# inai17ibar/video-diffusion-pipeline-parallel

Measured on AMD Instinct MI355X. Metric: steady-state videos/sec (whole node), SVD 14f x 25step, higher is better.
Workload: dtype f16

## Files before the change

### include/svdpipe.h

```cpp
#ifndef SVDPIPE_H
#define SVDPIPE_H

#include <stddef.h>
#include <stdint.h>

#ifdef __cplusplus
extern "C" {
#endif

#define SP_OK 0
#define SP_EINVAL (-1)
#define SP_ELAUNCH (-2)

const char *sp_last_error(void);
int sp_version(void);
#define SP_ZERO_PAGE_BYTES 4096

enum { SP_A_LINEAR = 0, SP_A_CONV3X3 = 1, SP_A_TEMPORAL3 = 2 };

typedef struct sp_gemm_desc {
  const void *a;
  int64_t lda;
  int mode;
  int cin;
// ... 33 lines not shown

const char *sp_gemm_last_kernel(void);

int sp_conv_up2x_f16(const void *a, int64_t lda, int cin, int n_img, int hin, int win, const void *w, int n,
                     const float *bias, void *d, int64_t ldd, float *gn_part, const void *zero_page, void *stream);

int sp_gemm_set_route(int route, int bm, int bn);

int sp_gemv_f16(const void *x, int64_t ldx, const void *w, const float *b, float *y, void *y_f16,
                int64_t ldy, int rows, int n, int k, int silu_in, int silu_out, void *stream);
int sp_gemv_batched_f16(const void *x, int64_t ldx, int64_t x_stride, const void *w, int64_t w_stride,
                        const float *b, int64_t b_stride, float *y, void *y_f16, int64_t ldy, int64_t y_stride,
                        int batch, int rows, int n, int k, int silu_in, int silu_out, void *stream);

int sp_sinusoid_f16(const float *values, void *out, int count, int dim, void *stream);

size_t sp_groupnorm_ws_bytes(int instances, int64_t rows, int c, int groups);
int sp_groupnorm_f16(const void *x, const float *gamma, const float *beta, void *y, int instances,
                     int64_t rows, int c, int groups, float eps, int fuse_silu, void *ws,
                     size_t ws_bytes, void *stream);
int sp_groupnorm_ld_f16(const void *x, int64_t ldx, const float *gamma, const float *beta, void *y, int instances,
                        int64_t rows, int c, int groups, float eps, int fuse_silu, void *ws,
                        size_t ws_bytes, void *stream);

int sp_groupnorm_tile_sums_f16(const void *x, int64_t ldx, const float *part, const float *gamma, const float *beta, void *y,
                               int instances, int64_t rows, int c, int groups, float eps, int fuse_silu, float *stats,
                               void *stream);
int sp_groupnorm_tile_sums2_f16(const void *x, int64_t ldx, const float *part, int c_a, const float *part_b, const float *gamma,
                                const float *beta, void *y, int instances, int64_t rows, int c, int groups, float eps,
                                int fuse_silu, float *stats, void *stream);
int sp_groupnorm_fold_linear_tile_sums_f16(const float *part, const float *gamma, const float *beta, int instances, int64_t rows,
                                           int c, int groups, float eps, const void *w, const float *bias, int n, void *w_out,
                                           float *bias_out, float *stats, void *stream);
int sp_groupnorm_fold_linear_f16(const void *x, int64_t ldx, const float *gamma, const float *beta, int instances,
                                 int64_t rows, int c, int groups, float eps, const void *w, const float *bias, int n,
                                 void *w_out, float *bias_out, void *ws, size_t ws_bytes, void *stream);

int sp_layernorm_f16(const void *x, const void *addvec, int64_t addvec_rows, void *sum_out,
                     const float *gamma, const float *beta, void *y, int64_t rows, int c, float eps,
                     void *stream);
int sp_ln_stats_f16(const void *x, const void *addvec, int64_t addvec_rows, void *sum_out, float *stats,
                    int64_t rows, int c, float eps, void *stream);

int sp_attn_spatial_f16(const void *q, const void *k, const void *v, void *o, int64_t ldq,
                        int64_t ldk, int64_t ldv, int64_t ldo, int batch, int seq, int heads,
                        float scale, const void *zero_page, void *stream);
int sp_attn_temporal_f16(const void *q, const void *k, const void *v, void *o, int64_t ldq,
                         int64_t ldk, int64_t ldv, int64_t ldo, int batch, int frames, int64_t hw,
                         int heads, float scale, const void *zero_page, void *stream);
int64_t sp_attn_long_ws_bytes(int batch, int seq, int heads);
int sp_attn_spatial_long_f16(const void *q, const void *k, const void *v, void *o, int64_t ldq, int64_t ldk,
                             int64_t ldv, int64_t ldo, int batch, int seq, int heads, float scale,
                             const void *zero_page, void *workspace, int64_t workspace_bytes, void *stream);
int64_t sp_attn_fp8_ws_bytes(int batch, int seq, int heads);
int sp_attn_spatial_fp8(const void *q, const void *k, const void *v, void *o, int64_t ldq, int64_t ldk,
                        int64_t ldv, int64_t ldo, int batch, int seq, int heads, float scale,
                        void *workspace, int64_t workspace_bytes, const void *zero_page, void *stream);

int sp_pack_input_f16(const void *latent, const void *image_latents, void *out, float in_scale,
                      int b, int frames, int h, int w, int cpad, void *stream);
int sp_euler_step_f16(const void *latent, const void *eps_cond, const void *eps_uncond,
                      int64_t ld_eps, const float *guidance , void *out, float sigma,
                      float sigma_next, int b, int frames, int h, int w, void *stream);
int sp_euler_step_rows_f16(const void *latent, const void *eps_cond, const void *eps_uncond,
                           int64_t ld_eps, const float *guidance, int64_t ld_guidance, void *out, float sigma,
                           float sigma_next, int b, int frames, int h, int w, void *stream);
int sp_dpmpp2m_step_rows_f16(const void *state, const void *eps_cond, const void *eps_uncond,
                             int64_t ld_eps, const float *guidance, int64_t ld_guidance, void *out_state,
                             float sigma, float a, float b, float c1, float c2,
                             int batch, int frames, int h, int w, void *stream);
int sp_concat_channels_f16(const void *a, int ca, const void *b, int cb, void *out, int64_t rows,
                           void *stream);
int sp_add_rowvec_f16(const void *x, const float *vec, void *y, int64_t rows, int c, void *stream);

int sp_softmax_rows_f16(void *x, int64_t ld, int64_t rows, int cols, void *stream);
int sp_gemm_f32out_f16(const void *a, int64_t lda, const void *w, void *d, int m, int n, int k, const void *zero_page,
                       void *stream);
int sp_softmax_rows_f32(const float *x, int64_t ld, void *out, int64_t ldo, int64_t rows, int cols, float scale, void *stream);
int sp_vae_pack_latent_f16(const void *latent, void *rows, float scale, int64_t flat0, int n, int F, int64_t sb,
                           int64_t sc, int64_t sf, int h, int w, int cpad, void *stream);
int sp_vae_frames_out_f16(const void *rows, int64_t ld, const float *weight, const float *bias, void *out,
                          int out_fp32, int batch, int frames, int h, int w, int64_t flat0, int F, int64_t sb,
                          int64_t sc, int64_t sf, void *stream);
int sp_vae_frames_out_u8(const void *rows, int64_t ld, const float *weight, const float *bias, void *out, int batch,
                         int frames, int h, int w, int64_t flat0, void *stream);

int sp_vae_image_pack_f16(const void *image, void *rows, int batch, int h, int w, int cpad, int flip, void *stream);
int sp_vae_latent_out_f16(const void *rows, int64_t ld, void *out, int batch, int channels, int frames, int h, int w,
                          int flip, void *stream);

int sp_patchify_f16(const void *pixels, void *rows, int batch, int h, int w, int patch, int kpad, void *stream);
int sp_attn_small_f16(const void *q, const void *k, const void *v, void *o, int64_t ldq, int64_t ldk, int64_t ldv,
                      int64_t ldo, int batch, int seq, int heads, int head_dim, float scale, void *stream);
int sp_gelu_f16(const void *x, void *y, int64_t n, int quick, void *stream);

enum { SP_FILTER_BICUBIC = 0 , SP_FILTER_LANCZOS3 = 1  };
size_t sp_image_resample_tmp_bytes(int src_h, int dst_w);
int sp_image_resample_u8(const void *src, int64_t src_pitch, int src_h, int src_w, void *dst, int64_t dst_pitch, int dst_h,
                         int dst_w, int filter, void *tmp, size_t tmp_bytes, void *stream);
int sp_image_to_tensor_f16(const void *src, int64_t src_pitch, int h, int w, void *out, float mean0, float mean1, float mean2,
                           float std0, float std1, float std2, void *stream);
int sp_frames_to_u8(const void *frames, int is_fp32, void *out, int batch, int frames_n, int h, int w, void *stream);

int sp_jpeg_quant_tables(int quality, uint8_t *luma64, uint8_t *chroma64);
int sp_jpeg_huffman_table(int which, uint8_t *bits16, uint8_t *vals162);
size_t sp_jpeg_coef_bytes(int n, int h, int w);
// ... 59 lines not shown
```

### video-diffusion-pipeline-parallel_amd/csrc/attention_long.hip

```cpp
#include "common.h"

namespace {

typedef unsigned u32x4 __attribute__((ext_vector_type(4)));
typedef unsigned u32x2 __attribute__((ext_vector_type(2)));

__device__ __forceinline__ float fast_exp2(float x) { return __builtin_amdgcn_exp2f(x); }

constexpr unsigned LONG_BAIL_MIN = 64, LONG_BAIL_MAX = 512;

template <int QB>
__global__ __launch_bounds__(256, 1) void attn_long_kernel(
    const f16 *__restrict__ q, const f16 *__restrict__ k, const f16 *__restrict__ v, f16 *__restrict__ o,
    int64_t ldq, int64_t ldk, int64_t ldv, int64_t ldo, int seq, int heads, float scale_log2e,
    unsigned *__restrict__ flags) {
  constexpr int KV = 64;
  constexpr int K_BYTES = KV * 128, STAGE = 2 * K_BYTES, RING = 3;
  constexpr int OWN = 2 * QB;
  constexpr int WARM = OWN + 1;
  __shared__ __attribute__((aligned(16))) char smem[RING * STAGE];

  const int tid = threadIdx.x, lane = tid & 63;
  const int wave = __builtin_amdgcn_readfirstlane(tid >> 6);
  const int bh = blockIdx.y;
  {
    unsigned *const flagged_waves = flags + (int64_t)gridDim.x * gridDim.y;
    if (tid == 0) *(volatile unsigned *)smem = __hip_atomic_load(flagged_waves, __ATOMIC_RELAXED, __HIP_MEMORY_SCOPE_AGENT);
    __syncthreads();
    const unsigned seen = *(volatile unsigned *)smem;
    __syncthreads();
    const unsigned total_waves = gridDim.x * gridDim.y * 4u;
    const unsigned frac = total_waves / 16u;
    const unsigned bail = frac < LONG_BAIL_MIN ? LONG_BAIL_MIN : (frac > LONG_BAIL_MAX ? LONG_BAIL_MAX : frac);
    if (seen >= bail) {
      if (tid == 0) flags[(int64_t)bh * gridDim.x + blockIdx.x] = 1u;
      return;
    }
  }
  const int b = bh / heads, hd = bh - b * heads;
  const int r = lane & 31, h = lane >> 5;
  const int64_t row0 = (int64_t)b * seq;
  const int q0 = blockIdx.x * (128 * QB) + wave * (32 * QB);

  f16x8 qf[QB][4];
#pragma unroll
  for (int qb = 0; qb < QB; ++qb) {
    const f16 *qp = q + (row0 + q0 + qb * 32 + r) * ldq + hd * 64 + 8 * h;
#pragma unroll
    for (int s = 0; s < 4; ++s) {
      const f16x8 raw = *(const f16x8 *)(qp + 16 * s);
#pragma unroll
      for (int e = 0; e < 8; ++e) qf[qb][s][e] = (f16)((float)raw[e] * scale_log2e);
    }
  }

  const int lrow = lane >> 3, lchunk = lane & 7;
  unsigned kofl[2], vofl[2];
#pragma unroll
  for (int i = 0; i < 2; ++i) {
    const int row = wave * 16 + i * 8 + lrow;
    kofl[i] = (unsigned)((row * ldk + ((lchunk ^ ((row >> 1) & 7)) << 3)) * 2);
    vofl[i] = (unsigned)((row * ldv + ((lchunk ^ (((row >> 1) & 1) << 2)) << 3)) * 2);
  }
  const int64_t kstep = (int64_t)KV * ldk * 2, vstep = (int64_t)KV * ldv * 2;

  int koff[2];
#pragma unroll
  for (int kt = 0; kt < 2; ++kt) koff[kt] = (kt * 32 + r) * 128;
  int kswz = (r >> 1) & 7, hq = h;
  const int g = lane >> 4, i16 = lane & 15, q_ = i16 >> 2, pp = i16 & 3;
  const int vrow_l = 4 * (g >> 1) + q_;
  const int vchunk_l = 2 * (g & 1) + (pp >> 1);
  const int vswz = (q_ >> 1) << 2;
// ... 23 lines not shown

  const int own0 = blockIdx.x * OWN;
  const char *kbase = (const char *)(k + row0 * ldk + hd * 64);
  const char *vbase = (const char *)(v + row0 * ldv + hd * 64);
  auto stage = [&](int i, int buf) {
    const int tl = i < OWN ? own0 + i : (i - OWN < own0 ? i - OWN : i);
    const char *kb = kbase + tl * kstep, *vb = vbase + tl * vstep;
    char *sk = smem + buf * STAGE;
    char *sv = sk + K_BYTES;
#pragma unroll
    for (int j = 0; j < 2; ++j) {
      glds16(kb + kofl[j], sk + (wave * 16 + j * 8) * 128);
      glds16(vb + vofl[j], sv + (wave * 16 + j * 8) * 128);
    }
  };
  stage(0, 0);
  stage(1, 1);
  asm volatile("s_waitcnt vmcnt(4)" ::: "memory");
  __builtin_amdgcn_s_barrier();

  auto qk = [&](int qb, const char *sk, f32x16 (&sacc)[2]) {
    f16x8 kf[2][4];
#pragma unroll
    for (int kt = 0; kt < 2; ++kt)
#pragma unroll
      for (int s = 0; s < 4; ++s) kf[kt][s] = *(const f16x8 *)(sk + koff[kt] + (((2 * s + hq) ^ kswz) << 4));
#pragma unroll
    for (int kt = 0; kt < 2; ++kt)
#pragma unroll
      for (int s = 0; s < 4; ++s)
        sacc[kt] = __builtin_amdgcn_mfma_f32_32x32x16_f16(kf[kt][s], qf[qb][s], s == 0 ? negm[qb] : sacc[kt], 0, 0, 0);
  };
  auto pv = [&](int qb, const u32x4 (&pw)[2][2], const u32x2 (&vr)[2][8]) {
#pragma unroll
    for (int dt = 0; dt < 2; ++dt)
#pragma unroll
      for (int kt = 0; kt < 2; ++kt)
#pragma unroll
        for (int s = 0; s < 2; ++s) {
          const u32x4 vw = {vr[dt][4 * kt + 2 * s][0], vr[dt][4 * kt + 2 * s][1], vr[dt][4 * kt + 2 * s + 1][0],
                            vr[dt][4 * kt + 2 * s + 1][1]};
          oacc[qb][dt] = __builtin_amdgcn_mfma_f32_32x32x16_f16(__builtin_bit_cast(f16x8, vw),
                                                               __builtin_bit_cast(f16x8, pw[kt][s]), oacc[qb][dt], 0, 0, 0);
          if (dt == 0)
            lacc[qb] = __builtin_amdgcn_mfma_f32_16x16x32_f16(lsel, __builtin_bit_cast(f16x8, pw[kt][s]), lacc[qb], 0, 0, 0);
        }
  };

  auto warm_tile = [&](int i, int buf) {
    if (i + 2 < ntiles) stage(i + 2, buf >= 1 ? buf - 1 : RING - 1);
    const char *sk = smem + buf * STAGE;
    const char *sv = sk + K_BYTES;

    f32x16 sacc[2][2];
    u32x4 pw[2][2][2];
    qk(0, sk, sacc[0]);
    u32x2 vr[2][8];
    {
      const unsigned va[2] = {(unsigned)(uintptr_t)(const __attribute__((address_space(3))) char *)(sv + vlane0),
                              (unsigned)(uintptr_t)(const __attribute__((address_space(3))) char *)(sv + vlane1)};
#pragma unroll
      for (int dt = 0; dt < 2; ++dt)
#pragma unroll
        for (int j = 0; j < 8; ++j)
          asm volatile("ds_read_b64_tr_b16 %0, %1 offset:%2" : "=v"(vr[dt][j]) : "v"(va[dt]), "n"(j * 8 * 128) : "memory");
      asm volatile("s_waitcnt lgkmcnt(0)"
                   : "+v"(vr[0][0]), "+v"(vr[0][1]), "+v"(vr[0][2]), "+v"(vr[0][3]), "+v"(vr[0][4]), "+v"(vr[0][5]),
                     "+v"(vr[0][6]), "+v"(vr[0][7]), "+v"(vr[1][0]), "+v"(vr[1][1]), "+v"(vr[1][2]), "+v"(vr[1][3]),
                     "+v"(vr[1][4]), "+v"(vr[1][5]), "+v"(vr[1][6]), "+v"(vr[1][7])::"memory");
    }

#pragma unroll
    for (int qb = 0; qb < QB; ++qb) {
      f32x16(&sc)[2] = sacc[qb & 1];
      if (qb > 0) pv(qb - 1, pw[(qb - 1) & 1], vr);
      {
        float mt = fmaxf(fmaxf(sc[0][0], sc[0][1]), sc[0][2]);
#pragma unroll
        for (int e = 3; e < 31; e += 2) mt = fmaxf(fmaxf(mt, sc[e >> 4][e & 15]), sc[(e + 1) >> 4][(e + 1) & 15]);
        mt = fmaxf(mt, sc[1][15]);
        float ma = mt, mb = mt;
        asm volatile("s_nop 1\n\tv_permlane32_swap_b32 %0, %1" : "+v"(ma), "+v"(mb));
        mt = fmaxf(ma, mb);
        const float delta = i == 0 ? mt : fmaxf(mt, 0.f);
        if (__builtin_amdgcn_ballot_w64(delta != 0.f) != 0) {
          const float alpha = i == 0 ? 1.f : fast_exp2(-delta);
          lacc[qb][0] *= alpha;
#pragma unroll
          for (int e = 0; e < 16; ++e) { oacc[qb][0][e] *= alpha; oacc[qb][1][e] *= alpha; }
#pragma unroll
          for (int kt = 0; kt < 2; ++kt)
#pragma unroll
            for (int e = 0; e < 16; ++e) sc[kt][e] -= delta;
          m_run[qb] += delta;
#pragma unroll
          for (int e = 0; e < 16; ++e) negm[qb][e] = -m_run[qb];
        }
      }
      if (qb + 1 < QB) qk(qb + 1, sk, sacc[(qb + 1) & 1]);
      u32x4(&pc)[2][2] = pw[qb & 1];
#pragma unroll
      for (int kt = 0; kt < 2; ++kt)
#pragma unroll
        for (int e = 0; e < 16; e += 2) {
          const f32x2 p = {fast_exp2(sc[kt][e]), fast_exp2(sc[kt][e + 1])};
          pc[kt][e >> 3][(e & 7) >> 1] = __builtin_bit_cast(unsigned, __builtin_convertvector(p, f16x2));
// ... 98 lines not shown
#pragma unroll
    for (int s = 0; s < 4; ++s) { S(1, 1, s); Q(0, 1, 0, s); RV(s); SB(); }
    asm volatile("s_waitcnt lgkmcnt(0)"
                 : "+v"(vr[0][0]), "+v"(vr[0][1]), "+v"(vr[0][2]), "+v"(vr[0][3]), "+v"(vr[1][0]), "+v"(vr[1][1]), "+v"(vr[1][2]),
                   "+v"(vr[1][3])::"memory");
    SB();
    STAMP(3);
    P(0, 0, 0, 0); Q(0, 1, 1, 0); RV(4); SB();
    P(0, 0, 0, 1); Q(0, 1, 1, 1); RV(5); SB();
    P(0, 0, 0, 2); Q(0, 1, 1, 2); RV(6); SB();
    P(0, 0, 1, 0); Q(0, 1, 1, 3); RV(7); SB();
    P(0, 0, 1, 1); SB();
    P(0, 0, 1, 2); SB();
    asm volatile("s_waitcnt lgkmcnt(0)"
                 : "+v"(vr[0][4]), "+v"(vr[0][5]), "+v"(vr[0][6]), "+v"(vr[0][7]), "+v"(vr[1][4]), "+v"(vr[1][5]), "+v"(vr[1][6]),
                   "+v"(vr[1][7])::"memory");
    SB();
    STAMP(4);
    asm volatile("s_waitcnt vmcnt(2)" ::: "memory");
    __builtin_amdgcn_s_barrier();
    SB();
    STAMP(5);
#define ROW(pb, pkt, ps, qkt, qs, X0, X1, X2)                              \
    P(pb, pkt, ps, 0); Q(1, qkt, qs, 0); Q(1, qkt, qs, 1); X0; SB();       \
    P(pb, pkt, ps, 1); Q(1, qkt, qs, 2); X1; SB();                         \
    P(pb, pkt, ps, 2); Q(1, qkt, qs, 3); X2; SB();
    ROW(0, 1, 0, 0, 0, dma(1, false), , )
    ROW(0, 1, 1, 0, 1, dma(1, true), , )
    STAMP(6);
    ROW(1, 0, 0, 1, 0, RK(0), RK(1), RK(2))
    ROW(1, 0, 1, 1, 1, RK(3), RK(4), RK(5))
#undef ROW
    STAMP(7);
    P(1, 1, 0, 0); RK(6); SB();
    P(1, 1, 0, 1); RK(7); SB();
    P(1, 1, 0, 2); advance_global(); SB();
    P(1, 1, 1, 0); SB();
    P(1, 1, 1, 1); advance_slots(); SB();
    P(1, 1, 1, 2); SB();
    STAMP(8);
#undef SB
#undef STAMP
  };

  int buf = 0;
  for (int i = 0; i < WARM; ++i) {
    warm_tile(i, buf);
    buf = buf + 1 == RING ? 0 : buf + 1;
  }
#pragma unroll
  for (int qb = 0; qb < QB; ++qb)
#pragma unroll
    for (int s = 0; s < 4; ++s) asm volatile("" : "+v"(qf[qb][s]));
  asm volatile("" : "+v"(koff[0]), "+v"(koff[1]), "+v"(vlane0), "+v"(vlane1), "+v"(kofl[0]), "+v"(kofl[1]), "+v"(vofl[0]),
               "+v"(vofl[1]), "+v"(lsel), "+v"(kswz), "+v"(hq));
  read_k(buf);
#ifdef LONG_TRACE
  const unsigned long long tc0 = __builtin_amdgcn_s_memtime(), tw0 = wall_clock64();
#endif
  steady_setup(WARM, buf);
  for (int i = WARM; i < ntiles; ++i) steady2(i);
  asm volatile("s_waitcnt vmcnt(0)" ::: "memory");

#ifdef LONG_TRACE
  tr[14] = (unsigned)(__builtin_amdgcn_s_memtime() - tc0);
  tr[15] = (unsigned)(wall_clock64() - tw0);
  if (blockIdx.x == 3 && blockIdx.y == LONG_TRACE && tid < 16) flags[gridDim.x * gridDim.y + 1 + tid] = tr[tid];
#endif
  {
    bool bad = false;
#pragma unroll
    for (int qb = 0; qb < QB; ++qb) bad = bad || !(lacc[qb][0] < 3.0e38f);
    if (__builtin_amdgcn_ballot_w64(bad) != 0 && lane == 0) {
      flags[(int64_t)bh * gridDim.x + blockIdx.x] = 1u;
      __hip_atomic_fetch_add(flags + (int64_t)gridDim.x * gridDim.y, 1u, __ATOMIC_RELAXED, __HIP_MEMORY_SCOPE_AGENT);
    }
  }

#pragma unroll
  for (int qb = 0; qb < QB; ++qb) {
    const float inv = 1.0f / lacc[qb][0];
    f16 *op = o + (row0 + q0 + qb * 32 + r) * ldo + hd * 64 + 4 * h;
#pragma unroll
    for (int dt = 0; dt < 2; ++dt)
#pragma unroll
      for (int c = 0; c < 4; ++c) {
        f16x4 w;
#pragma unroll
        for (int e = 0; e < 4; ++e) w[e] = (f16)(oacc[qb][dt][4 * c + e] * inv);
        *(f16x4 *)(op + 32 * dt + 8 * c) = w;
      }
  }
}

}

constexpr int LONG_QB = 2;
constexpr int LONG_ROWS = 128 * LONG_QB;

int sp_attn_spatial_launch(const void *q, const void *k, const void *v, void *o, int64_t ldq, int64_t ldk, int64_t ldv,
                           int64_t ldo, int batch, int seq, int heads, float scale, const void *zero_page,
                           const unsigned *only_flagged, void *stream, const char *who);

extern "C" int64_t sp_attn_long_ws_bytes(int batch, int seq, int heads) {
  if (batch <= 0 || seq <= 0 || heads <= 0) return 0;
  return ((int64_t)batch * heads * ((seq + LONG_ROWS - 1) / LONG_ROWS) + 1) * (int64_t)sizeof(unsigned);
}

extern "C" int sp_attn_spatial_long_f16(const void *q, const void *k, const void *v, void *o, int64_t ldq, int64_t ldk,
                                        int64_t ldv, int64_t ldo, int batch, int seq, int heads, float scale,
                                        const void *zero_page, void *workspace, int64_t workspace_bytes, void *stream) {
  SP_REQUIRE(q && k && v && o && zero_page, "sp_attn_spatial_long_f16: null pointer");
  SP_REQUIRE(batch > 0 && seq > 0 && heads > 0, "sp_attn_spatial_long_f16: batch/seq/heads must be positive");
  if (!(seq >= 4096 && seq % LONG_ROWS == 0))
    return sp_attn_spatial_launch(q, k, v, o, ldq, ldk, ldv, ldo, batch, seq, heads, scale, zero_page, nullptr, stream,
                                  "sp_attn_spatial_long_f16");
  SP_REQUIRE(ldq % 8 == 0 && ldk % 8 == 0 && ldv % 8 == 0 && ldo % 4 == 0,
             "sp_attn_spatial_long_f16: strides must be multiples of 8");
  SP_REQUIRE((int64_t)batch * heads <= 65535, "sp_attn_spatial_long_f16: batch*heads too large");
  const int64_t need = sp_attn_long_ws_bytes(batch, seq, heads);
  SP_REQUIRE(workspace && ((uintptr_t)workspace & 3) == 0 && workspace_bytes >= need,
             "sp_attn_spatial_long_f16: workspace of %lld bytes, need %lld (4-byte aligned)", (long long)workspace_bytes,
             (long long)need);
  SP_REQUIRE(5 * 64 * ldk * 2 < (1ll << 31) && 5 * 64 * ldv * 2 < (1ll << 31), "sp_attn_spatial_long_f16: row stride too large");
  hipStream_t s = (hipStream_t)stream;
  unsigned *flags = (unsigned *)workspace;
  if (hipMemsetAsync(flags, 0, (size_t)need, s) != hipSuccess) {
    (void)hipGetLastError();
    sp_set_error("sp_attn_spatial_long_f16: hipMemsetAsync of the flag words failed");
    return SP_ELAUNCH;
  }
  SP_CLEAR_STALE_ERROR();
  hipLaunchKernelGGL(attn_long_kernel<LONG_QB>, dim3(seq / LONG_ROWS, batch * heads), dim3(256), 0, s, (const f16 *)q,
                     (const f16 *)k, (const f16 *)v, (f16 *)o, ldq, ldk, ldv, ldo, seq, heads, scale * 1.4426950408889634f,
                     flags);
  SP_CHECK_LAUNCH("sp_attn_spatial_long_f16");
  return sp_attn_spatial_launch(q, k, v, o, ldq, ldk, ldv, ldo, batch, seq, heads, scale, zero_page, flags, stream,
                                "sp_attn_spatial_long_f16(second pass)");
}
```

### video-diffusion-pipeline-parallel_amd/hip/__init__.py

```python

from __future__ import annotations

import ctypes
import os

_HERE = os.path.dirname(os.path.abspath(__file__))
LIB_PATH = os.path.join(_HERE, "libsvdpipe_hip.so")
_lib = None


class GemmDesc(ctypes.Structure):

    _fields_ = [
        ("a", ctypes.c_void_p), ("lda", ctypes.c_int64), ("mode", ctypes.c_int), ("cin", ctypes.c_int),
        ("n_img", ctypes.c_int), ("hin", ctypes.c_int), ("win", ctypes.c_int), ("hout", ctypes.c_int),
        ("wout", ctypes.c_int), ("stride", ctypes.c_int), ("upsample2x", ctypes.c_int),
        ("frames", ctypes.c_int), ("hw", ctypes.c_int64),
        ("w", ctypes.c_void_p), ("m", ctypes.c_int), ("n", ctypes.c_int),
        ("bias", ctypes.c_void_p), ("bias2", ctypes.c_void_p), ("bias2_rows", ctypes.c_int64),
        ("ldb2", ctypes.c_int64),
        ("res1", ctypes.c_void_p), ("ldr1", ctypes.c_int64), ("r1scale", ctypes.c_float),
        ("res2", ctypes.c_void_p), ("ldr2", ctypes.c_int64), ("r2scale", ctypes.c_float),
        ("oscale", ctypes.c_float), ("geglu", ctypes.c_int), ("n_store", ctypes.c_int),
        ("d", ctypes.c_void_p), ("ldd", ctypes.c_int64), ("zero_page", ctypes.c_void_p),
        ("ln_stats", ctypes.c_void_p), ("ln_colsum", ctypes.c_void_p),
        ("euler_latent", ctypes.c_void_p), ("euler_out", ctypes.c_void_p),
        ("euler_eps_uncond", ctypes.c_void_p), ("euler_ld_eps", ctypes.c_int64),
        ("euler_guidance", ctypes.c_void_p),
        ("euler_sigma", ctypes.c_float), ("euler_sigma_next", ctypes.c_float),
        ("euler_frames", ctypes.c_int), ("euler_hw", ctypes.c_int64),
        ("workspace", ctypes.c_void_p), ("workspace_bytes", ctypes.c_size_t),
        ("ln_out", ctypes.c_void_p), ("ln_out_eps", ctypes.c_float),
        ("w_group_rows", ctypes.c_int64), ("w_group_stride", ctypes.c_int64),
        ("gn_part", ctypes.c_void_p),
        ("a2", ctypes.c_void_p), ("lda2", ctypes.c_int64), ("cin2", ctypes.c_int),
        ("euler_guidance_ld", ctypes.c_int64),
    ]


_P, _I, _L, _F, _Z = ctypes.c_void_p, ctypes.c_int, ctypes.c_int64, ctypes.c_float, ctypes.c_size_t
SIGNATURES = {
    "sp_last_error": (ctypes.c_char_p, []),
    "sp_version": (_I, []),
    "sp_gemm_f16": (_I, [ctypes.POINTER(GemmDesc), _P]),
    "sp_gemm_desc_size": (_Z, []),
    "sp_gemm_workspace_bytes": (_Z, [ctypes.POINTER(GemmDesc)]),
    "sp_gemm_set_route": (_I, [_I, _I, _I]),
    "sp_gemm_last_kernel": (ctypes.c_char_p, []),
    "sp_conv_up2x_f16": (_I, [_P, _L, _I, _I, _I, _I, _P, _I, _P, _P, _L, _P, _P, _P]),
    "sp_gemv_f16": (_I, [_P, _L, _P, _P, _P, _P, _L, _I, _I, _I, _I, _I, _P]),
    "sp_gemv_batched_f16": (_I, [_P, _L, _L, _P, _L, _P, _L, _P, _P, _L, _L, _I, _I, _I, _I, _I, _I, _P]),
    "sp_sinusoid_f16": (_I, [_P, _P, _I, _I, _P]),
    "sp_groupnorm_ws_bytes": (_Z, [_I, _L, _I, _I]),
    "sp_groupnorm_f16": (_I, [_P, _P, _P, _P, _I, _L, _I, _I, _F, _I, _P, _Z, _P]),
    "sp_groupnorm_ld_f16": (_I, [_P, _L, _P, _P, _P, _I, _L, _I, _I, _F, _I, _P, _Z, _P]),
    "sp_groupnorm_tile_sums_f16": (_I, [_P, _L, _P, _P, _P, _P, _I, _L, _I, _I, _F, _I, _P, _P]),
    "sp_groupnorm_tile_sums2_f16": (_I, [_P, _L, _P, _I, _P, _P, _P, _P, _I, _L, _I, _I, _F, _I, _P, _P]),
    "sp_groupnorm_fold_linear_tile_sums_f16": (_I, [_P, _P, _P, _I, _L, _I, _I, _F, _P, _P, _I, _P, _P, _P, _P]),
    "sp_groupnorm_fold_linear_f16": (_I, [_P, _L, _P, _P, _I, _L, _I, _I, _F, _P, _P, _I, _P, _P, _P, _Z, _P]),
    "sp_layernorm_f16": (_I, [_P, _P, _L, _P, _P, _P, _P, _L, _I, _F, _P]),
    "sp_ln_stats_f16": (_I, [_P, _P, _L, _P, _P, _L, _I, _F, _P]),
    "sp_attn_spatial_f16": (_I, [_P, _P, _P, _P, _L, _L, _L, _L, _I, _I, _I, _F, _P, _P]),
    "sp_attn_long_ws_bytes": (_L, [_I, _I, _I]),
    "sp_attn_spatial_long_f16": (_I, [_P, _P, _P, _P, _L, _L, _L, _L, _I, _I, _I, _F, _P, _P, _L, _P]),
    "sp_attn_fp8_ws_bytes": (_L, [_I, _I, _I]),
    "sp_attn_spatial_fp8": (_I, [_P, _P, _P, _P, _L, _L, _L, _L, _I, _I, _I, _F, _P, _L, _P, _P]),
    "sp_attn_temporal_f16": (_I, [_P, _P, _P, _P, _L, _L, _L, _L, _I, _I, _L, _I, _F, _P, _P]),
    "sp_pack_input_f16": (_I, [_P, _P, _P, _F, _I, _I, _I, _I, _I, _P]),
    "sp_euler_step_f16": (_I, [_P, _P, _P, _L, _P, _P, _F, _F, _I, _I, _I, _I, _P]),
    "sp_euler_step_rows_f16": (_I, [_P, _P, _P, _L, _P, _L, _P, _F, _F, _I, _I, _I, _I, _P]),
    "sp_dpmpp2m_step_rows_f16": (_I, [_P, _P, _P, _L, _P, _L, _P, _F, _F, _F, _F, _F, _I, _I, _I, _I, _P]),
    "sp_concat_channels_f16": (_I, [_P, _I, _P, _I, _P, _L, _P]),
    "sp_add_rowvec_f16": (_I, [_P, _P, _P, _L, _I, _P]),
    "sp_softmax_rows_f16": (_I, [_P, _L, _L, _I, _P]),
    "sp_gemm_f32out_f16": (_I, [_P, _L, _P, _P, _I, _I, _I, _P, _P]),
    "sp_softmax_rows_f32": (_I, [_P, _L, _P, _L, _L, _I, _F, _P]),
    "sp_vae_pack_latent_f16": (_I, [_P, _P, _F, _L, _I, _I, _L, _L, _L, _I, _I, _I, _P]),
    "sp_vae_frames_out_f16": (_I, [_P, _L, _P, _P, _P, _I, _I, _I, _I, _I, _L, _I, _L, _L, _L, _P]),
    "sp_vae_frames_out_u8": (_I, [_P, _L, _P, _P, _P, _I, _I, _I, _I, _L, _P]),
    "sp_vae_image_pack_f16": (_I, [_P, _P, _I, _I, _I, _I, _I, _P]),
    "sp_vae_latent_out_f16": (_I, [_P, _L, _P, _I, _I, _I, _I, _I, _I, _P]),
    "sp_patchify_f16": (_I, [_P, _P, _I, _I, _I, _I, _I, _P]),
    "sp_attn_small_f16": (_I, [_P, _P, _P, _P, _L, _L, _L, _L, _I, _I, _I, _I, _F, _P]),
    "sp_gelu_f16": (_I, [_P, _P, _L, _I, _P]),
    "sp_image_resample_tmp_bytes": (_Z, [_I, _I]),
    "sp_image_resample_u8": (_I, [_P, _L, _I, _I, _P, _L, _I, _I, _I, _P, _Z, _P]),
    "sp_image_to_tensor_f16": (_I, [_P, _L, _I, _I, _P, _F, _F, _F, _F, _F, _F, _P]),
    "sp_frames_to_u8": (_I, [_P, _I, _P, _I, _I, _I, _I, _P]),
    "sp_jpeg_quant_tables": (_I, [_I, _P, _P]),
    "sp_jpeg_huffman_table": (_I, [_I, _P, _P]),
    "sp_jpeg_coef_bytes": (_Z, [_I, _I, _I]),
    "sp_jpeg_dct_quant_u8": (_I, [_P, _I, _I, _I, _I, _P, _P]),
    "sp_jpeg_stream_bytes": (_Z, [_I, _I, _I]),
    "sp_jpeg_entropy_ws_bytes": (_Z, [_I, _I, _I, _I]),
    "sp_jpeg_entropy": (_I, [_P, _I, _I, _I, _I, _P, _Z, _P, _P, _Z, _P]),
    "sp_jpeg_decode_plan_bytes": (_Z, []),
    "sp_jpeg_decode_plan": (_I, [_P, _P, _I, _P, _P, _I, _P]),
    "sp_jpeg_decode_ws_bytes": (_Z, [_P]),
    "sp_jpeg_decode_coef_bytes": (_Z, [_P]),
    "sp_jpeg_decode_split": (_I, [_P, _P, _P, _P, _Z, _P]),
    "sp_jpeg_decode_sync": (_I, [_P, _P, _P, _Z, _I, _I, _P]),
    "sp_jpeg_decode_coefficients": (_I, [_P, _P, _P, _Z, _I, _P, _P]),
    "sp_jpeg_decode_pixels": (_I, [_P, _P, _P, _Z, _P, _P, _P]),
    "sp_gif_ws_bytes": (_Z, [_I, _I, _I, _I]),
    "sp_gif_stream_bytes": (_Z, [_I, _I, _I]),
    "sp_gif_quantise_u8": (_I, [_P, _I, _I, _I, _P, _P, _P, _Z, _P]),
    "sp_gif_lzw": (_I, [_P, _I, _I, _I, _I, _P, _Z, _P, _P, _Z, _P]),
    "sp_png_ws_bytes": (_Z, [_I, _I, _I, _I]),
    "sp_png_stream_bytes": (_Z, [_I, _I, _I]),
    "sp_png_filter_u8": (_I, [_P, _I, _I, _I, _P, _P]),
    "sp_png_deflate": (_I, [_P, _I, _I, _I, _I, _P, _Z, _P, _P, _Z, _P]),
    "sp_png_file_bytes": (_Z, [_I, _I, _I]),
    "sp_apng_file_bytes": (_Z, [_I, _I, _I, _I]),
    "sp_png_wrap_ws_bytes": (_Z, [_I, _Z]),
    "sp_png_wrap": (_I, [_P, _Z, _P, _I, _I, _I, _I, _I, _I, _P, _Z, _P, _P, _Z, _P]),
    "sp_crc32_ws_bytes": (_Z, [_I, _Z]),
    "sp_crc32_rows": (_I, [_P, _Z, _P, _P, _I, _P, _P, _Z, _P]),
# ... 35 lines not shown
```

### video-diffusion-pipeline-parallel_amd/hip/ops.py

```python

from __future__ import annotations

import ctypes

import torch

from . import GemmDesc, last_error, load

A_LINEAR, A_CONV3X3, A_TEMPORAL3 = 0, 1, 2
ZERO_PAGE_BYTES = 4096
_zero_pages: dict = {}


class HipKernelError(RuntimeError):
    pass


PROFILE = None


class _Timed:
    def __init__(self, kind, flops, nbytes=0.0, tag=None):
        self.kind, self.flops, self.nbytes, self.tag = kind, flops, nbytes, tag

# ... 207 lines not shown


def groupnorm_fold_linear(x, gamma, beta, w, bias, w_out, bias_out, *, instances, rows, c, groups, eps, n, ws, ldx=None):
    with _Timed("groupnorm", 0.0, 2.0 * instances * rows * c + 2.0 * instances * n * c):
        ldx = int(c if ldx is None else ldx)
        if tuple(w_out.shape) != (instances, n, c) or not w_out.is_contiguous() or bias_out.dtype != torch.float32 \
                or tuple(bias_out.shape) != (instances, n) or not bias_out.is_contiguous():
            raise ValueError("groupnorm_fold_linear: w_out must be contiguous fp16 [instances][n][c], bias_out fp32 [instances][n]")
        _check(load().sp_groupnorm_fold_linear_f16(_rows(x, "x", ldx).data_ptr(), ldx, _ptr(gamma), _ptr(beta), instances,
                                                   rows, c, groups, eps, _f16(w, "w").data_ptr(), _ptr(bias), n,
                                                   _f16(w_out, "w_out").data_ptr(), bias_out.data_ptr(), ws.data_ptr(),
                                                   ws.numel() * ws.element_size(), _stream()), "sp_groupnorm_fold_linear_f16")
    return w_out, bias_out


def layernorm(x, gamma, beta, y, *, rows, c, eps=1e-5, addvec=None, addvec_rows=0, sum_out=None):
    with _Timed("layernorm", 0.0, (2 + (sum_out is not None)) * 2.0 * rows * c):
        _check(load().sp_layernorm_f16(_f16(x, "x").data_ptr(), _ptr(addvec), addvec_rows, _ptr(sum_out),
                                       gamma.data_ptr(), beta.data_ptr(), _f16(y, "y").data_ptr(), rows, c, eps,
                                       _stream()), "sp_layernorm_f16")
    return y


def ln_stats(x, stats, *, rows, c, eps=1e-5, addvec=None, addvec_rows=0, sum_out=None):
    with _Timed("ln_stats", 0.0, (1 + (sum_out is not None)) * 2.0 * rows * c + 8.0 * rows):
        _check(load().sp_ln_stats_f16(_f16(x, "x").data_ptr(), _ptr(addvec), addvec_rows, _ptr(sum_out),
                                      stats.data_ptr(), rows, c, eps, _stream()), "sp_ln_stats_f16")
    return stats


def attn_spatial(q, k, v, o, *, ldq, ldk, ldv, ldo, batch, seq, heads, scale=0.125):
    with _Timed("attn_spatial", 4.0 * batch * heads * seq * seq * 64):
        _check(load().sp_attn_spatial_f16(q.data_ptr(), k.data_ptr(), v.data_ptr(), o.data_ptr(), ldq, ldk, ldv, ldo,
                                          batch, seq, heads, scale, zero_page(o.device).data_ptr(), _stream()),
               "sp_attn_spatial_f16")
    return o


def attn_long_ws_bytes(batch, seq, heads) -> int:
    return int(load().sp_attn_long_ws_bytes(batch, seq, heads))


def attn_spatial_long(q, k, v, o, workspace, *, ldq, ldk, ldv, ldo, batch, seq, heads, scale=0.125):
    long_rows = seq >= 4096 and seq % 256 == 0
    with _Timed("attn_spatial_long" if long_rows else "attn_spatial", 4.0 * batch * heads * seq * seq * 64):
        _check(load().sp_attn_spatial_long_f16(q.data_ptr(), k.data_ptr(), v.data_ptr(), o.data_ptr(), ldq, ldk, ldv, ldo,
                                               batch, seq, heads, scale, zero_page(o.device).data_ptr(),
                                               workspace.data_ptr(), workspace.numel() * workspace.element_size(),
                                               _stream()),
               "sp_attn_spatial_long_f16")
    return o


def attn_fp8_ws_bytes(batch, seq, heads) -> int:
    return int(load().sp_attn_fp8_ws_bytes(batch, seq, heads))


def attn_spatial_fp8(q, k, v, o, workspace, *, ldq, ldk, ldv, ldo, batch, seq, heads, scale=0.125):
    with _Timed("attn_spatial", 4.0 * batch * heads * seq * seq * 64):
        _check(load().sp_attn_spatial_fp8(q.data_ptr(), k.data_ptr(), v.data_ptr(), o.data_ptr(), ldq, ldk, ldv, ldo,
                                          batch, seq, heads, scale, workspace.data_ptr(),
                                          workspace.numel() * workspace.element_size(),
                                          zero_page(o.device).data_ptr(), _stream()),
               "sp_attn_spatial_fp8")
    return o


def attn_temporal(q, k, v, o, *, ldq, ldk, ldv, ldo, batch, frames, hw, heads, scale=0.125):
    with _Timed("attn_temporal", 4.0 * batch * hw * heads * frames * frames * 64, 4 * 2.0 * batch * frames * hw * heads * 64):
        _check(load().sp_attn_temporal_f16(q.data_ptr(), k.data_ptr(), v.data_ptr(), o.data_ptr(), ldq, ldk, ldv, ldo,
                                           batch, frames, hw, heads, scale, zero_page(o.device).data_ptr(), _stream()),
               "sp_attn_temporal_f16")
    return o


def pack_input(latent, image_latents, out, *, in_scale, b, frames, h, w, cpad):
    _check(load().sp_pack_input_f16(_f16(latent, "latent").data_ptr(), _f16(image_latents, "image_latents").data_ptr(),
                                    out.data_ptr(), in_scale, b, frames, h, w, cpad, _stream()), "sp_pack_input_f16")
    return out


def softmax_rows(x, *, rows, cols, ld=None):
    ld = int(ld if ld is not None else cols)
    with _Timed("softmax_rows", 0.0, 2 * 2.0 * rows * cols):
        _check(load().sp_softmax_rows_f16(_rows(x, "x", ld).data_ptr(), ld, rows, cols, _stream()), "sp_softmax_rows_f16")
    return x


def gemm_f32out(a, w, out32, *, m, n, k, lda=None):
    lda = int(lda if lda is not None else a.stride(0))
    _f16(a, "a"); _f16(w, "w")
    if out32.dtype != torch.float32 or not out32.is_cuda or not out32.is_contiguous() or out32.numel() < m * n:
        raise TypeError("out32 must be a contiguous float32 HIP tensor of at least m*n elements")
    if w.dim() == 2 and w.shape[0] > 1 and w.stride(0) != k:
        raise ValueError(f"w: row stride {w.stride(0)} must equal k = {k}")
    with _Timed("gemm_f32out", 2.0 * m * n * k, 2.0 * (m * k + n * k) + 4.0 * m * n):
        _check(load().sp_gemm_f32out_f16(a.data_ptr(), lda, w.data_ptr(), out32.data_ptr(), m, n, k,
                                         zero_page(a.device).data_ptr(), _stream()), "sp_gemm_f32out_f16")
    return out32


def softmax_rows_f32(x32, out16, *, rows, cols, scale=1.0, ld=None, ldo=None):
    ld = int(ld if ld is not None else x32.stride(0))
    ldo = int(ldo if ldo is not None else out16.stride(0))
    if x32.dtype != torch.float32 or not x32.is_cuda or out16.dtype != torch.float16 or not out16.is_cuda:
        raise TypeError("x32 must be float32 and out16 float16, both on a HIP device")
# ... 504 lines not shown
```

Before: 0.8371.

## Run long spatial attention at two waves per SIMD with periodic early-bail checks

Templates the long attention kernel on occupancy and by default launches a variant with launch_bounds occupancy 2. That variant uses a simpler warm-up tile path, and every 32 tiles it checks for overflow and for the global bail counter so blocks can quit early to the fallback pass. The aim is to hide latency through more resident waves per SIMD, at the cost of tighter register budgets and a less hand-scheduled pipeline. It also adds a setter for the occupancy mode and a query that reports which kernel was last launched.

```diff
diff --git a/include/svdpipe.h b/include/svdpipe.h
--- a/include/svdpipe.h
+++ b/include/svdpipe.h
@@ -109,6 +109,8 @@
 int sp_attn_spatial_long_f16(const void *q, const void *k, const void *v, void *o, int64_t ldq, int64_t ldk,
                              int64_t ldv, int64_t ldo, int batch, int seq, int heads, float scale,
                              const void *zero_page, void *workspace, int64_t workspace_bytes, void *stream);
+int sp_attn_long_set_occupancy(int occ);
+const char *sp_attn_long_last_kernel(void);
 int64_t sp_attn_fp8_ws_bytes(int batch, int seq, int heads);
 int sp_attn_spatial_fp8(const void *q, const void *k, const void *v, void *o, int64_t ldq, int64_t ldk,
                         int64_t ldv, int64_t ldo, int batch, int seq, int heads, float scale,
diff --git a/video-diffusion-pipeline-parallel_amd/csrc/attention_long.hip b/video-diffusion-pipeline-parallel_amd/csrc/attention_long.hip
--- a/video-diffusion-pipeline-parallel_amd/csrc/attention_long.hip
+++ b/video-diffusion-pipeline-parallel_amd/csrc/attention_long.hip
@@ -8,9 +8,10 @@
 __device__ __forceinline__ float fast_exp2(float x) { return __builtin_amdgcn_exp2f(x); }
 
 constexpr unsigned LONG_BAIL_MIN = 64, LONG_BAIL_MAX = 512;
-
-template <int QB>
-__global__ __launch_bounds__(256, 1) void attn_long_kernel(
+constexpr int LONG_LOOK = 32;
+
+template <int QB, int OCC>
+__global__ __launch_bounds__(256, OCC) void attn_long_kernel(
     const f16 *__restrict__ q, const f16 *__restrict__ k, const f16 *__restrict__ v, f16 *__restrict__ o,
     int64_t ldq, int64_t ldk, int64_t ldv, int64_t ldo, int seq, int heads, float scale_log2e,
     unsigned *__restrict__ flags) {
@@ -18,7 +19,7 @@
   constexpr int K_BYTES = KV * 128, STAGE = 2 * K_BYTES, RING = 3;
   constexpr int OWN = 2 * QB;
   constexpr int WARM = OWN + 1;
-  __shared__ __attribute__((aligned(16))) char smem[RING * STAGE];
+  __shared__ __attribute__((aligned(16))) char smem[RING * STAGE + (OCC > 1 ? 32 : 0)];
 
   const int tid = threadIdx.x, lane = tid & 63;
   const int wave = __builtin_amdgcn_readfirstlane(tid >> 6);
@@ -148,6 +149,60 @@
     const char *sk = smem + buf * STAGE;
     const char *sv = sk + K_BYTES;
 
+    if constexpr (OCC > 1) {
+#pragma unroll
+      for (int qb = 0; qb < QB; ++qb) {
+        f32x16 sc[2];
+        qk(qb, sk, sc);
+        u32x2 vr[2][8];
+        {
+          const unsigned va[2] = {(unsigned)(uintptr_t)(const __attribute__((address_space(3))) char *)(sv + vlane0),
+                                  (unsigned)(uintptr_t)(const __attribute__((address_space(3))) char *)(sv + vlane1)};
+#pragma unroll
+          for (int dt = 0; dt < 2; ++dt)
+#pragma unroll
+            for (int j = 0; j < 8; ++j)
+              asm volatile("ds_read_b64_tr_b16 %0, %1 offset:%2" : "=v"(vr[dt][j]) : "v"(va[dt]), "n"(j * 8 * 128) : "memory");
+          asm volatile("s_waitcnt lgkmcnt(0)"
+                       : "+v"(vr[0][0]), "+v"(vr[0][1]), "+v"(vr[0][2]), "+v"(vr[0][3]), "+v"(vr[0][4]), "+v"(vr[0][5]),
+                         "+v"(vr[0][6]), "+v"(vr[0][7]), "+v"(vr[1][0]), "+v"(vr[1][1]), "+v"(vr[1][2]), "+v"(vr[1][3]),
+                         "+v"(vr[1][4]), "+v"(vr[1][5]), "+v"(vr[1][6]), "+v"(vr[1][7])::"memory");
+        }
+        float mt = fmaxf(fmaxf(sc[0][0], sc[0][1]), sc[0][2]);
+#pragma unroll
+        for (int e = 3; e < 31; e += 2) mt = fmaxf(fmaxf(mt, sc[e >> 4][e & 15]), sc[(e + 1) >> 4][(e + 1) & 15]);
+        mt = fmaxf(mt, sc[1][15]);
+        float ma = mt, mb = mt;
+        asm volatile("s_nop 1\n\tv_permlane32_swap_b32 %0, %1" : "+v"(ma), "+v"(mb));
+        mt = fmaxf(ma, mb);
+        const float delta = i == 0 ? mt : fmaxf(mt, 0.f);
+        if (__builtin_amdgcn_ballot_w64(delta != 0.f) != 0) {
+          const float alpha = i == 0 ? 1.f : fast_exp2(-delta);
+          lacc[qb][0] *= alpha;
+#pragma unroll
+          for (int e = 0; e < 16; ++e) { oacc[qb][0][e] *= alpha; oacc[qb][1][e] *= alpha; }
+#pragma unroll
+          for (int kt = 0; kt < 2; ++kt)
+#pragma unroll
+            for (int e = 0; e < 16; ++e) sc[kt][e] -= delta;
+          m_run[qb] += delta;
+#pragma unroll
+          for (int e = 0; e < 16; ++e) negm[qb][e] = -m_run[qb];
+        }
+        u32x4 pc[2][2];
+#pragma unroll
+        for (int kt = 0; kt < 2; ++kt)
+#pragma unroll
+          for (int e = 0; e < 16; e += 2) {
+            const f32x2 p = {fast_exp2(sc[kt][e]), fast_exp2(sc[kt][e + 1])};
+            pc[kt][e >> 3][(e & 7) >> 1] = __builtin_bit_cast(unsigned, __builtin_convertvector(p, f16x2));
+          }
+        pv(qb, pc, vr);
+      }
+      if (i + 2 < ntiles) asm volatile("s_waitcnt vmcnt(4)" ::: "memory"); else asm volatile("s_waitcnt vmcnt(0)" ::: "memory");
+      __builtin_amdgcn_s_barrier();
+      return;
+    }
     f32x16 sacc[2][2];
     u32x4 pw[2][2][2];
     qk(0, sk, sacc[0]);
@@ -352,6 +407,10 @@
   for (int qb = 0; qb < QB; ++qb)
 #pragma unroll
     for (int s = 0; s < 4; ++s) asm volatile("" : "+v"(qf[qb][s]));
+  if constexpr (OCC > 1) {
+    const int ln = (int)__builtin_amdgcn_mbcnt_hi(~0u, __builtin_amdgcn_mbcnt_lo(~0u, 0u));
+    kswz = ((ln & 31) >> 1) & 7; hq = ln >> 5;
+  }
   asm volatile("" : "+v"(koff[0]), "+v"(koff[1]), "+v"(vlane0), "+v"(vlane1), "+v"(kofl[0]), "+v"(kofl[1]), "+v"(vofl[0]),
                "+v"(vofl[1]), "+v"(lsel), "+v"(kswz), "+v"(hq));
   read_k(buf);
@@ -359,7 +418,48 @@
   const unsigned long long tc0 = __builtin_amdgcn_s_memtime(), tw0 = wall_clock64();
 #endif
   steady_setup(WARM, buf);
-  for (int i = WARM; i < ntiles; ++i) steady2(i);
+  if constexpr (OCC > 1) {
+    volatile __attribute__((address_space(3))) unsigned *const look =
+        (volatile __attribute__((address_space(3))) unsigned *)(__attribute__((address_space(3))) char *)(smem + RING * STAGE);
+    bool quit = false;
+    for (int i = WARM; i < ntiles && !quit;) {
+      const int stop = i + LONG_LOOK < ntiles ? i + LONG_LOOK : ntiles;
+      for (; i < stop; ++i) steady2(i);
+      if (i < ntiles) {
+        bool bad = false;
+#pragma unroll
+        for (int qb = 0; qb < QB; ++qb) bad = bad || !(lacc[qb][0] < 3.0e38f);
+        const bool wave_bad = __builtin_amdgcn_ballot_w64(bad) != 0;
+        const int ln = (int)__builtin_amdgcn_mbcnt_hi(~0u, __builtin_amdgcn_mbcnt_lo(~0u, 0u));
+        if (ln == 0) {
+          look[wave] = wave_bad ? 1u : 0u;
+          if (wave == 0)
+            look[4] = __hip_atomic_load(flags + (int64_t)gridDim.x * gridDim.y, __ATOMIC_RELAXED, __HIP_MEMORY_SCOPE_AGENT);
+        }
+        asm volatile("s_waitcnt lgkmcnt(0)" ::: "memory");
+        __builtin_amdgcn_s_barrier();
+        const unsigned any_bad = look[0] | look[1] | look[2] | look[3], seen = look[4];
+        const unsigned total_waves = gridDim.x * gridDim.y * 4u;
+        const unsigned frac = total_waves / 16u;
+        const unsigned bail = frac < LONG_BAIL_MIN ? LONG_BAIL_MIN : (frac > LONG_BAIL_MAX ? LONG_BAIL_MAX : frac);
+        quit = __builtin_amdgcn_readfirstlane(any_bad != 0 || seen >= bail);
+      }
+    }
+    if (quit) {
+      asm volatile("s_waitcnt vmcnt(0)" ::: "memory");
+      bool bad = false;
+#pragma unroll
+      for (int qb = 0; qb < QB; ++qb) bad = bad || !(lacc[qb][0] < 3.0e38f);
+      const bool wave_bad = __builtin_amdgcn_ballot_w64(bad) != 0;
+      const int ln = (int)__builtin_amdgcn_mbcnt_hi(~0u, __builtin_amdgcn_mbcnt_lo(~0u, 0u));
+      if (ln == 0 && (wave == 0 || wave_bad)) flags[(int64_t)bh * gridDim.x + blockIdx.x] = 1u;
+      if (ln == 0 && wave_bad)
+        __hip_atomic_fetch_add(flags + (int64_t)gridDim.x * gridDim.y, 1u, __ATOMIC_RELAXED, __HIP_MEMORY_SCOPE_AGENT);
+      return;
+    }
+  } else {
+    for (int i = WARM; i < ntiles; ++i) steady2(i);
+  }
   asm volatile("s_waitcnt vmcnt(0)" ::: "memory");
 
 #ifdef LONG_TRACE
@@ -367,11 +467,16 @@
   tr[15] = (unsigned)(wall_clock64() - tw0);
   if (blockIdx.x == 3 && blockIdx.y == LONG_TRACE && tid < 16) flags[gridDim.x * gridDim.y + 1 + tid] = tr[tid];
 #endif
+  int lane_t = lane, r_t = r, h_t = h;
+  if constexpr (OCC > 1) {
+    lane_t = (int)__builtin_amdgcn_mbcnt_hi(~0u, __builtin_amdgcn_mbcnt_lo(~0u, 0u));
+    r_t = lane_t & 31; h_t = lane_t >> 5;
+  }
   {
     bool bad = false;
 #pragma unroll
     for (int qb = 0; qb < QB; ++qb) bad = bad || !(lacc[qb][0] < 3.0e38f);
-    if (__builtin_amdgcn_ballot_w64(bad) != 0 && lane == 0) {
+    if (__builtin_amdgcn_ballot_w64(bad) != 0 && lane_t == 0) {
       flags[(int64_t)bh * gridDim.x + blockIdx.x] = 1u;
       __hip_atomic_fetch_add(flags + (int64_t)gridDim.x * gridDim.y, 1u, __ATOMIC_RELAXED, __HIP_MEMORY_SCOPE_AGENT);
     }
@@ -380,7 +485,7 @@
 #pragma unroll
   for (int qb = 0; qb < QB; ++qb) {
     const float inv = 1.0f / lacc[qb][0];
-    f16 *op = o + (row0 + q0 + qb * 32 + r) * ldo + hd * 64 + 4 * h;
+    f16 *op = o + (row0 + q0 + qb * 32 + r_t) * ldo + hd * 64 + 4 * h_t;
 #pragma unroll
     for (int dt = 0; dt < 2; ++dt)
 #pragma unroll
@@ -396,6 +501,9 @@
 }
 
 constexpr int LONG_QB = 2;
+constexpr int LONG_OCC_DEFAULT = 2;
+static int g_long_occ = 0;
+static thread_local const char *g_long_last = "";
 constexpr int LONG_ROWS = 128 * LONG_QB;
 
 int sp_attn_spatial_launch(const void *q, const void *k, const void *v, void *o, int64_t ldq, int64_t ldk, int64_t ldv,
@@ -406,15 +514,24 @@
   if (batch <= 0 || seq <= 0 || heads <= 0) return 0;
   return ((int64_t)batch * heads * ((seq + LONG_ROWS - 1) / LONG_ROWS) + 1) * (int64_t)sizeof(unsigned);
 }
+
+extern "C" int sp_attn_long_set_occupancy(int occ) {
+  SP_REQUIRE(occ >= 0 && occ <= 2, "sp_attn_long_set_occupancy: occ %d (0 default, 1 or 2 waves per SIMD)", occ);
+  g_long_occ = occ;
+  return SP_OK;
+}
+extern "C" const char *sp_attn_long_last_kernel(void) { return g_long_last; }
 
 extern "C" int sp_attn_spatial_long_f16(const void *q, const void *k, const void *v, void *o, int64_t ldq, int64_t ldk,
                                         int64_t ldv, int64_t ldo, int batch, int seq, int heads, float scale,
                                         const void *zero_page, void *workspace, int64_t workspace_bytes, void *stream) {
   SP_REQUIRE(q && k && v && o && zero_page, "sp_attn_spatial_long_f16: null pointer");
   SP_REQUIRE(batch > 0 && seq > 0 && heads > 0, "sp_attn_spatial_long_f16: batch/seq/heads must be positive");
-  if (!(seq >= 4096 && seq % LONG_ROWS == 0))
+  if (!(seq >= 4096 && seq % LONG_ROWS == 0)) {
+    g_long_last = "attn_spatial_kernel";
     return sp_attn_spatial_launch(q, k, v, o, ldq, ldk, ldv, ldo, batch, seq, heads, scale, zero_page, nullptr, stream,
                                   "sp_attn_spatial_long_f16");
+  }
   SP_REQUIRE(ldq % 8 == 0 && ldk % 8 == 0 && ldv % 8 == 0 && ldo % 4 == 0,
              "sp_attn_spatial_long_f16: strides must be multiples of 8");
   SP_REQUIRE((int64_t)batch * heads <= 65535, "sp_attn_spatial_long_f16: batch*heads too large");
@@ -431,9 +548,17 @@
     return SP_ELAUNCH;
   }
   SP_CLEAR_STALE_ERROR();
-  hipLaunchKernelGGL(attn_long_kernel<LONG_QB>, dim3(seq / LONG_ROWS, batch * heads), dim3(256), 0, s, (const f16 *)q,
-                     (const f16 *)k, (const f16 *)v, (f16 *)o, ldq, ldk, ldv, ldo, seq, heads, scale * 1.4426950408889634f,
-                     flags);
+  const dim3 grid(seq / LONG_ROWS, batch * heads);
+  const float scale_log2e = scale * 1.4426950408889634f;
+  if ((g_long_occ ? g_long_occ : LONG_OCC_DEFAULT) == 2) {
+    g_long_last = "attn_long_kernel<2, 2>";
+    hipLaunchKernelGGL((attn_long_kernel<LONG_QB, 2>), grid, dim3(256), 0, s, (const f16 *)q, (const f16 *)k, (const f16 *)v,
+                       (f16 *)o, ldq, ldk, ldv, ldo, seq, heads, scale_log2e, flags);
+  } else {
+    g_long_last = "attn_long_kernel<2, 1>";
+    hipLaunchKernelGGL((attn_long_kernel<LONG_QB, 1>), grid, dim3(256), 0, s, (const f16 *)q, (const f16 *)k, (const f16 *)v,
+                       (f16 *)o, ldq, ldk, ldv, ldo, seq, heads, scale_log2e, flags);
+  }
   SP_CHECK_LAUNCH("sp_attn_spatial_long_f16");
   return sp_attn_spatial_launch(q, k, v, o, ldq, ldk, ldv, ldo, batch, seq, heads, scale, zero_page, flags, stream,
                                 "sp_attn_spatial_long_f16(second pass)");
diff --git a/video-diffusion-pipeline-parallel_amd/hip/__init__.py b/video-diffusion-pipeline-parallel_amd/hip/__init__.py
--- a/video-diffusion-pipeline-parallel_amd/hip/__init__.py
+++ b/video-diffusion-pipeline-parallel_amd/hip/__init__.py
@@ -63,6 +63,8 @@
     "sp_attn_spatial_f16": (_I, [_P, _P, _P, _P, _L, _L, _L, _L, _I, _I, _I, _F, _P, _P]),
     "sp_attn_long_ws_bytes": (_L, [_I, _I, _I]),
     "sp_attn_spatial_long_f16": (_I, [_P, _P, _P, _P, _L, _L, _L, _L, _I, _I, _I, _F, _P, _P, _L, _P]),
+    "sp_attn_long_set_occupancy": (_I, [_I]),
+    "sp_attn_long_last_kernel": (ctypes.c_char_p, []),
     "sp_attn_fp8_ws_bytes": (_L, [_I, _I, _I]),
     "sp_attn_spatial_fp8": (_I, [_P, _P, _P, _P, _L, _L, _L, _L, _I, _I, _I, _F, _P, _L, _P, _P]),
     "sp_attn_temporal_f16": (_I, [_P, _P, _P, _P, _L, _L, _L, _L, _I, _I, _L, _I, _F, _P, _P]),
diff --git a/video-diffusion-pipeline-parallel_amd/hip/ops.py b/video-diffusion-pipeline-parallel_amd/hip/ops.py
--- a/video-diffusion-pipeline-parallel_amd/hip/ops.py
+++ b/video-diffusion-pipeline-parallel_amd/hip/ops.py
@@ -283,6 +283,14 @@
     return o
 
 
+def attn_long_set_occupancy(occ: int) -> None:
+    _check(load().sp_attn_long_set_occupancy(occ), "sp_attn_long_set_occupancy")
+
+
+def attn_long_last_kernel() -> str:
+    return load().sp_attn_long_last_kernel().decode()
+
+
 def attn_fp8_ws_bytes(batch, seq, heads) -> int:
     return int(load().sp_attn_fp8_ws_bytes(batch, seq, heads))
 
```

After: 0.8553 (median of 6 runs). 1.02x the previous value.
